# YPares/gaast

Measured on AMD Instinct MI355X. Metric: full-MV geometric products/sec (dim n); achieved HBM GB/s vs roofline, higher is better.
Workload: dtype f32; 1 GPU; R^12 full MV x MV geometric product, f32 (BASELINE configs[2]); dim=12, batch_per_gpu=65536, global_batch=65536

## Files before the change

gaast_amd/csrc/device/kernels_dense.hip.hpp:

```cpp
#pragma once
#include "kernels_common.hip.hpp"


namespace gaast {

template <typename T>
struct DenseArgs {
    const T* left;
    const T* right;
    T* out;
    int64_t left_stride, right_stride, out_stride;
    const uint32_t* left_map;
    const uint32_t* right_map;
    int left_count, right_count;
    int left_full, right_full;
    int left_contig, right_contig;
    const int32_t* out_map;
    int canon_left, canon_right;
    int n;
    uint32_t neg_hi, zero_hi;
    uint32_t neg_lo;
    int beta;
    const T* left_scale;
    const T* right_scale;
    const T* out_scale;
    const T* pre_left;
    const T* pre_right;
    int64_t pre_left_stride, pre_right_stride;
    int pre_left_len, pre_right_len, pre_canon_left, pre_canon_right;
    const uint32_t* pre_row_start;
    const uint32_t* pre_entries;
    const T* pre_coeff;
    const uint32_t* pre_row_map;
    const T* pre_row_scale;
    int pre_rows;
    int pre_width;
    int pre_scratch;
    int left_signs;
    int out_signs;
    int64_t batch;
};

__device__ __forceinline__ int dense_lds_pos(int m) {
    const int x = m >> 4, lo = m & 15;
    return (x << 4) | ((((lo >> 2) ^ (x >> 2)) & 3) << 2) | (lo & 3);
}


__device__ __forceinline__ void split_index(int e, int cnt, float inv_cnt, int nitems, int& it, int& j) {
    if (nitems == 1) {
        it = 0;
        j = e;
        return;
    }
    int q = int(float(e) * inv_cnt);
    int r = e - q * cnt;
    if (r < 0) {
        --q;
        r += cnt;
    }
    if (r >= cnt) {
        ++q;
        r -= cnt;
    }
    it = q;
    j = r;
}

template <typename T, int THREADS>
__device__ __forceinline__ void stage_operands(const T* __restrict__ src, int64_t stride, const uint32_t* __restrict__ map,
                                               int count, int contig4, int canon, T* __restrict__ images,
                                               int image_stride, int nitems, int tid, const T* __restrict__ scale = nullptr) {
    constexpr int U = 4;
    const float inv_count = 1.0f / float(count > 0 ? count : 1);
    if (contig4) {
        const int total4 = (nitems * count) >> 2;
        const int count4 = count >> 2;
        const float inv_count4 = 1.0f / float(count4 > 0 ? count4 : 1);
        for (int e0 = tid; e0 < total4; e0 += THREADS * U) {
            uint4 m[U];
            T v[U][4];
#pragma unroll
            for (int k = 0; k < U; ++k) {
                const int e = e0 + k * THREADS;
// ... 439 lines not shown
        float16v acc;
#pragma unroll
        for (int r = 0; r < 16; ++r) acc[r] = 0.f;

        const unsigned char* As_b = reinterpret_cast<const unsigned char*>(As);
        const unsigned char* Bs_b = reinterpret_cast<const unsigned char*>(Bs);
        uint32_t bq[4];
#pragma unroll
        for (int q = 0; q < 4; ++q) bq[q] = (uint32_t(c_hi) << 7) | (uint32_t((((h << 2) | q) ^ (c_hi >> 1)) & 7) << 4);
        const uint32_t c_hi_u = uint32_t(c_hi) | 0x8000u;
        auto one_step = [&](int a_hi) {
            uint32_t sp = uint32_t(a_hi) >> 1;
            sp ^= sp >> 1;
            sp ^= sp >> 2;
            sp ^= sp >> 4;
            sp ^= sp >> 8;
            const uint32_t M = sp ^ (uint32_t(a_hi) & p.neg_hi);
            const uint32_t u = (__builtin_popcount(uint32_t(a_hi) & sp) ^
                                __builtin_popcount(uint32_t(a_hi) & p.neg_hi)) & 1u;
            const uint32_t bmask = uint32_t(__builtin_popcount(c_hi_u & (M | (u << 15)))) << 31;
            float bscale = 1.f;
            if (DEGENERATE) {
                if (uint32_t(a_hi) & ~uint32_t(c_hi) & p.zero_hi) bscale = 0.f;
            }
            float bv[16];
            const uint32_t sx = (uint32_t(a_hi) << 7) | (uint32_t((a_hi >> 1) & 7) << 4);
#pragma unroll
            for (int q = 0; q < 4; ++q) {
                const float4v v = *reinterpret_cast<const float4v*>(Bs_b + (bq[q] ^ sx));
                bv[4 * q + 0] = v.x; bv[4 * q + 1] = v.y; bv[4 * q + 2] = v.z; bv[4 * q + 3] = v.w;
            }
            const uint32_t abase = uint32_t(a_hi) << 7;
#pragma unroll
            for (int s2 = 0; s2 < 16; ++s2) {
                float a = *reinterpret_cast<const float*>(As_b + abase + aoff[s2]);
                a = __uint_as_float(__float_as_uint(a) ^ amask[s2]);
                float b = __uint_as_float(__float_as_uint(bv[s2]) ^ bmask);
                if (DEGENERATE) b *= bscale;
                acc = __builtin_amdgcn_mfma_f32_32x32x2f32(a, b, acc, 0, 0, 0);
            }
        };
        const int half = H >> 1;
        for (int t2 = 0; t2 < half; ++t2) one_step((t2 << 1) | (__builtin_popcount(uint32_t(t2)) & 1));
#pragma unroll
        for (int s2 = 0; s2 < 16; ++s2)
            amask[s2] ^= uint32_t((__builtin_popcount(uint32_t(s2)) + h) & 1) << 31;
        for (int t2 = 0; t2 < half; ++t2) one_step((t2 << 1) | ((__builtin_popcount(uint32_t(t2)) & 1) ^ 1));

        float* orow = p.out + (item0 + it) * p.out_stride;
        const int32_t* om = p.out_map + (c_hi << 5);
#pragma unroll
        for (int r = 0; r < 16; ++r) {
            const int c_lo = (r & 3) + 8 * (r >> 2) + 4 * h;
            store_result<float>(orow, om[c_lo], acc[r], p.beta, out_scale, (c_hi << 5) + c_lo);
        }
    }
}

template <int THREADS>
__device__ __forceinline__ void lds_barrier() {
    if (THREADS <= 64) {
        __builtin_amdgcn_wave_barrier();
        asm volatile("" ::: "memory");
    } else {
        asm volatile("s_waitcnt lgkmcnt(0)\n\ts_barrier" ::: "memory");
    }
}

typedef __attribute__((address_space(3))) unsigned char lds_u8;
typedef uint32_t uint4v __attribute__((ext_vector_type(4)));

__device__ __forceinline__ uint32_t xor3(uint32_t a, uint32_t b, uint32_t c) {
#if __has_builtin(__builtin_amdgcn_bitop3_b32)
    return __builtin_amdgcn_bitop3_b32(a, b, c, 0x96);
#else
    return a ^ b ^ c;
#endif
}

__device__ __forceinline__ constexpr int mfma16_k(int t) {
    constexpr int order[16] = {0, 3, 5, 6, 9, 10, 12, 15, 1, 2, 4, 7, 8, 11, 13, 14};
    return order[t];
}

template <bool DEGENERATE, int NDIM, bool SCALED = false, bool CHAINED = false>
__global__ __launch_bounds__(NDIM == 13 ? 512 : 256, NDIM <= 11 ? 2 : 1) void k_gp_mfma32p(DenseArgs<float> p) {
    const float* const left_scale = SCALED ? p.left_scale : nullptr;
    const float* const right_scale = SCALED ? p.right_scale : nullptr;
    const float* const out_scale = SCALED ? p.out_scale : nullptr;
    extern __shared__ __attribute__((aligned(16))) unsigned char smem_raw[];
    float* smem = reinterpret_cast<float*>(smem_raw);
    lds_u8* lds = (lds_u8*)smem_raw;
    constexpr int n = NDIM;
    constexpr int THREADS = NDIM == 13 ? 512 : 256;
    constexpr int N = 1 << n;
    constexpr int H = 1 << (n - 5);
    constexpr int WPI = H >> 5;
    constexpr int IPB = (THREADS >> 6) / WPI;
    constexpr int item_stride = 4 * N;
    constexpr uint32_t NEG = uint32_t(N) << 2;
    constexpr int PR = N / 4;
    constexpr int MPR = PR / THREADS;
    constexpr int ROWS = 2 * IPB;
    static_assert(MPR * ROWS == 8, "eight 16-byte pieces per thread and group");
    const int tid = threadIdx.x;
    const int64_t num_groups = (p.batch + IPB - 1) / IPB;
    const bool fast = !SCALED && !CHAINED && p.left_contig && p.right_contig && p.left_full && p.right_full;

    if (tid < 16) smem[IPB * item_stride + tid] = 0.f;

    uint32_t mw[2][MPR * 4];
    float4 pf[8];
    auto fetch = [&](int64_t g) {
        const int64_t it0 = g * IPB;
        const int cnt = int(p.batch - it0 < IPB ? p.batch - it0 : IPB);
#pragma unroll
        for (int r = 0; r < ROWS; ++r) {
            const int k = r % IPB;
            if (k < cnt) {
                const float* row = r < IPB ? p.left + (it0 + k) * p.left_stride : p.right + (it0 + k) * p.right_stride;
#pragma unroll
                for (int m = 0; m < MPR; ++m) pf[r * MPR + m] = reinterpret_cast<const float4*>(row)[tid + m * THREADS];
            }
        }
    };
    if (fast) {
#pragma unroll
        for (int m = 0; m < MPR; ++m) {
            const uint4 ml = reinterpret_cast<const uint4*>(p.left_map)[tid + m * THREADS];
            const uint4 mr = reinterpret_cast<const uint4*>(p.right_map)[tid + m * THREADS];
            mw[0][4 * m + 0] = ml.x; mw[0][4 * m + 1] = ml.y; mw[0][4 * m + 2] = ml.z; mw[0][4 * m + 3] = ml.w;
            mw[1][4 * m + 0] = mr.x; mw[1][4 * m + 1] = mr.y; mw[1][4 * m + 2] = mr.z; mw[1][4 * m + 3] = mr.w;
        }
        if (int64_t(blockIdx.x) < num_groups) fetch(blockIdx.x);
    }

    const int wave = tid >> 6, lane = tid & 63;
    const int it = wave / WPI, tile = wave - it * WPI;
    const int i = lane & 31, h = lane >> 5;
    const int c_hi = (tile << 5) | i;
    const uint32_t item_base = uint32_t(it) * uint32_t(item_stride) * 4u;

    constexpr bool ABS_A = NDIM <= 11 || (NDIM == 12 && !DEGENERATE);
    const uint32_t lds0 = ABS_A ? uint32_t(size_t(lds)) : 0u;
    uint32_t ak0[16];
#pragma unroll
    for (int t = 0; t < 16; ++t) {
        const int k = 2 * mfma16_k(t) + h;
        const int a_lo = i ^ k;
        int par = __builtin_popcount(uint32_t(a_lo & k) & p.neg_lo) & 1;
        for (int pp = 1; pp < 5; ++pp)
            if ((a_lo >> pp) & 1) par ^= __builtin_popcount(k & ((1 << pp) - 1)) & 1;
        ak0[t] = lds0 + item_base + (uint32_t(a_lo) << 2) + (par ? NEG : 0u);
    }
    const uint32_t b_base = item_base + 2u * NEG;
    constexpr uint32_t zero_block = uint32_t(IPB) * uint32_t(item_stride) * 4u;
    uint32_t bq[4];
#pragma unroll
    for (int q = 0; q < 4; ++q) {
        bq[q] = (uint32_t(c_hi) << 7) | (uint32_t((((h << 2) | q) ^ (c_hi >> 1)) & 7) << 4);
        if ((__builtin_popcount(uint32_t(c_hi)) & 1) && (((q >> 1) ^ h) & 1)) bq[q] ^= NEG;
    }
    const uint32_t c_hi_u = uint32_t(c_hi) | 0x8000u;
    auto sign_terms = [&](int a_hi, uint32_t& M, uint32_t& u) {
        uint32_t sp = uint32_t(a_hi) >> 1;
        sp ^= sp >> 1;
        sp ^= sp >> 2;
        sp ^= sp >> 4;
        sp ^= sp >> 8;
        M = sp ^ (uint32_t(a_hi) & p.neg_hi);
        u = (__builtin_popcount(uint32_t(a_hi) & sp) ^ __builtin_popcount(uint32_t(a_hi) & p.neg_hi)) & 1u;
    };
    auto block_sign = [&](int a_hi) -> uint32_t {
        uint32_t M, u;
        sign_terms(a_hi, M, u);
        return uint32_t(__builtin_popcount(c_hi_u & (M | (u << 15)))) & 1u;
    };
    constexpr int SIGN_WORDS = H <= 64 ? H / 32 : 0;
    constexpr bool XOR_STEP = NDIM == 12 && !DEGENERATE;
    if (XOR_STEP && (lds0 & ((16u << n) - 1u))) __builtin_trap();
    uint32_t dlt[XOR_STEP ? 7 : 1] = {0};
    uint32_t ud[XOR_STEP ? H / 32 : 1] = {0};
    if constexpr (XOR_STEP) {
#pragma unroll
        for (int t = 0; t < 7; ++t) {
            const uint32_t P = (2u << t) - 1u;
            uint32_t M, u;
            sign_terms(int(P), M, u);
            dlt[t] = (P << 7) ^ (((P >> 1) & 7u) << 4) ^ ((uint32_t(__builtin_popcount(uint32_t(c_hi) & M)) & 1u) << (n + 2));
        }
#pragma unroll
        for (int w = 0; w < H / 32; ++w) {
            uint32_t bits = 0;
#pragma unroll 1
            for (int b = 0; b < 32; ++b) {
                uint32_t M, u0, u1;
                sign_terms(32 * w + b, M, u0);
                sign_terms(32 * w + b + 1, M, u1);
                bits |= (u0 ^ u1) << b;
            }
            ud[w] = __builtin_amdgcn_readfirstlane(bits);
        }
    }
    uint32_t sgn[SIGN_WORDS > 0 ? SIGN_WORDS : 1] = {0};
#pragma unroll
    for (int w = 0; w < SIGN_WORDS; ++w) {
        uint32_t bits = 0;
#pragma unroll 1
        for (int b = 0; b < 32; ++b) bits |= block_sign(32 * w + b) << b;
        sgn[w] = bits;
    }

    for (int64_t g = blockIdx.x; g < num_groups; g += gridDim.x) {
        const int64_t item0 = g * IPB;
        const int nitems = int(p.batch - item0 < IPB ? p.batch - item0 : IPB);
        if (fast) {
            auto stage_row = [&](int r, bool canon) {
                const int k = r % IPB, side = r / IPB;
                if (k < nitems) {
#pragma unroll
                    for (int m = 0; m < MPR; ++m) {
                        const float4 v = pf[r * MPR + m];
                        const float x[4] = {v.x, v.y, v.z, v.w};
#pragma unroll
                        for (int c = 0; c < 4; ++c) {
                            const uint32_t w = mw[side][4 * m + c];
                            float y = x[c];
                            if (canon) y = 0.f + y;
                            const uint32_t yb = __float_as_uint(y) ^ (w & 0x80000000u);
                            const uint32_t at = uint32_t(k) * uint32_t(item_stride * 4) + (side ? 2u * NEG : 0u) + (((w >> 16) & 0x7fffu) << 2);
                            *(__attribute__((address_space(3))) uint32_t*)(lds + at) = yb;
                            *(__attribute__((address_space(3))) uint32_t*)(lds + at + NEG) = yb ^ 0x80000000u;
                        }
                    }
                }
            };
#pragma unroll
            for (int r = 0; r < ROWS; ++r) {
                if constexpr (XOR_STEP) {
                    if (r / IPB ? p.canon_right : p.canon_left) stage_row(r, true);
                    else stage_row(r, false);
                } else {
                    stage_row(r, r / IPB ? p.canon_right : p.canon_left);
                }
            }
        } else {
            if (!p.left_full || !p.right_full) {
                for (int e = tid; e < nitems * item_stride; e += THREADS) smem[e] = 0.f;
                lds_barrier<THREADS>();
            }
            if constexpr (CHAINED)
                stage_from_list<float, THREADS>(p, item0, nitems, smem, item_stride, smem + p.pre_scratch, tid);
            else
                stage_operands<float, THREADS>(p.left + item0 * p.left_stride, p.left_stride, p.left_map, p.left_count, p.left_contig,
                                           p.canon_left, smem, item_stride, nitems, tid, left_scale);
            stage_operands<float, THREADS>(p.right + item0 * p.right_stride, p.right_stride, p.right_map, p.right_count,
                                           p.right_contig, p.canon_right, smem + 2 * N, item_stride, nitems, tid, right_scale);
            lds_barrier<THREADS>();
            constexpr int quads_per_item = N >> 1;
            for (int e = tid; e < nitems * quads_per_item; e += THREADS) {
                const int sit = e / quads_per_item, j = e - sit * quads_per_item;
                const int src = sit * item_stride + (j << 2) + ((j << 2) < N ? 0 : N);
                const float4v v = *reinterpret_cast<const float4v*>(smem + src);
                *reinterpret_cast<float4v*>(smem + src + N) = -v;
            }
        }
        lds_barrier<THREADS>();
        if (fast && g + gridDim.x < num_groups) fetch(g + gridDim.x);

        if (it < nitems) {
            float16v acc;
#pragma unroll
            for (int r = 0; r < 16; ++r) acc[r] = 0.f;
            uint32_t akc[XOR_STEP ? 1 : 16];
            uint32_t (&ak)[16] = *reinterpret_cast<uint32_t (*)[16]>(XOR_STEP ? ak0 : akc);
            if constexpr (!XOR_STEP) {
#pragma unroll
                for (int t = 0; t < 16; ++t) ak[t] = ak0[t];
            }

            auto step = [&](int a_hi, int j, uint32_t sxs) {
                uint32_t bw[16], aw[16];
#pragma unroll
                for (int q = 0; q < 4; ++q) {
                    uint32_t addr = b_base + (bq[q] ^ sxs);
                    if (DEGENERATE) addr = (uint32_t(a_hi) & ~uint32_t(c_hi) & p.zero_hi) ? zero_block : addr;
                    const uint4v v = *(__attribute__((address_space(3))) const uint4v*)(lds + addr);
                    bw[4 * q + 0] = v.x; bw[4 * q + 1] = v.y; bw[4 * q + 2] = v.z; bw[4 * q + 3] = v.w;
                }
#pragma unroll
                for (int t = 0; t < 16; ++t)
                    aw[t] = ABS_A ? *(__attribute__((address_space(3))) const uint32_t*)size_t(ak[t] + uint32_t(j << 7))
                                  : *(__attribute__((address_space(3))) const uint32_t*)(lds + ak[t] + uint32_t(j << 7));
#pragma unroll
                for (int t = 0; t < 16; ++t)
                    acc = __builtin_amdgcn_mfma_f32_32x32x2f32(__uint_as_float(aw[t]), __uint_as_float(bw[t]), acc, 0, 0, 0);
                asm volatile("" ::: "memory");
            };
            if constexpr (SIGN_WORDS > 0 && NDIM <= 11) {
                uint32_t awin[4];
                uint4v qb[2];
                auto b_quad = [&](int a_hi, int q, uint32_t sxs) -> uint4v {
                    uint32_t addr = b_base + (bq[q] ^ sxs);
                    if (DEGENERATE) addr = (uint32_t(a_hi) & ~uint32_t(c_hi) & p.zero_hi) ? zero_block : addr;
                    return *(__attribute__((address_space(3))) const uint4v*)(lds + addr);
                };
                auto a_word = [&](int t, int j) -> uint32_t {
                    return ABS_A ? *(__attribute__((address_space(3))) const uint32_t*)size_t(ak[t] + uint32_t(j << 7))
                                 : *(__attribute__((address_space(3))) const uint32_t*)(lds + ak[t] + uint32_t(j << 7));
                };
                auto sx_of = [&](int a_hi) -> uint32_t {
                    uint32_t sx = __builtin_amdgcn_readfirstlane((uint32_t(a_hi) << 7) | (uint32_t((a_hi >> 1) & 7) << 4));
                    asm("" : "+s"(sx));
                    return sx;
                };
                uint32_t sxs = ((sgn[0] & 1u) << (n + 2)) | sx_of(0);
                qb[0] = b_quad(0, 0, sxs);
#pragma unroll
                for (int t = 0; t < 3; ++t) awin[t] = a_word(t, 0);
#pragma unroll
                for (int w = 0; w < SIGN_WORDS; ++w) {
                    uint32_t sw = sgn[w];
                    const uint32_t next_word_bit0 = w + 1 < SIGN_WORDS ? (sgn[w + 1 < SIGN_WORDS ? w + 1 : w] & 1u) : 0u;
#pragma unroll 1
                    for (int c = 0; c < 2; ++c) {
                        const int a0 = 32 * w + 16 * c;
#pragma unroll
                        for (int j = 0; j < 16; ++j) {
                            const int a_hi = a0 + j;
                            const uint32_t nbit = j < 15 ? (sw >> (j + 1)) & 1u : (c == 0 ? (sw >> 16) & 1u : next_word_bit0);
                            const uint32_t nsxs = (nbit << (n + 2)) | sx_of(a_hi + 1);
#pragma unroll
                            for (int t = 0; t < 16; ++t) {
                                const int m = 16 * j + t;
                                const int t3 = (t + 3) & 15, j3 = j + ((t + 3) >> 4);
                                awin[(m + 3) & 3] = a_word(t3, j3);
                                if ((t & 3) == 0) {
                                    const int q = t >> 2;
                                    qb[(q + 1) & 1] = q < 3 ? b_quad(a_hi, q + 1, sxs) : b_quad(a_hi + 1, 0, nsxs);
                                }
                                __builtin_amdgcn_sched_barrier(0);
                                const uint4v bqv = qb[(t >> 2) & 1];
                                const uint32_t bwv = (t & 3) == 0 ? bqv.x : (t & 3) == 1 ? bqv.y : (t & 3) == 2 ? bqv.z : bqv.w;
                                acc = __builtin_amdgcn_mfma_f32_32x32x2f32(__uint_as_float(awin[m & 3]), __uint_as_float(bwv), acc, 0, 0, 0);
                                __builtin_amdgcn_sched_barrier(0);
                            }
                            sxs = nsxs;
                        }
                        sw >>= 16;
#pragma unroll
                        for (int t = 0; t < 16; ++t) ak[t] += 16u << 7;
                    }
                }
            } else if constexpr (XOR_STEP) {
                uint32_t xb[4];
#pragma unroll
                for (int q = 0; q < 4; ++q) xb[q] = lds0 + (b_base | bq[q]);
#pragma unroll 1
                for (int c = 0; c < H / 64; ++c) {
                    const uint32_t udw[2] = {c == 0 ? ud[0] : ud[2], c == 0 ? ud[1] : ud[3]};
#pragma unroll
                    for (int j = 0; j < 64; ++j) {
                        uint32_t bw[16], aw[16];
#pragma unroll
                        for (int q = 0; q < 4; ++q) {
                            const uint4v v = *(__attribute__((address_space(3))) const uint4v*)size_t(xb[q]);
                            bw[4 * q + 0] = v.x; bw[4 * q + 1] = v.y; bw[4 * q + 2] = v.z; bw[4 * q + 3] = v.w;
                        }
#pragma unroll
                        for (int t = 0; t < 16; ++t)
                            aw[t] = *(__attribute__((address_space(3))) const uint32_t*)size_t(ak[t] + uint32_t(j << 7));
#pragma unroll
                        for (int t = 0; t < 16; ++t)
                            acc = __builtin_amdgcn_mfma_f32_32x32x2f32(__uint_as_float(aw[t]), __uint_as_float(bw[t]), acc, 0, 0, 0);
                        asm volatile("" ::: "memory");
                        uint32_t su = __builtin_amdgcn_readfirstlane(((udw[j >> 5] >> (j & 31)) & 1u) << (n + 2));
                        asm("" : "+s"(su));
                        const uint32_t d = dlt[j < 63 ? __builtin_ctz(~uint32_t(j)) : 6];
#pragma unroll
                        for (int q = 0; q < 4; ++q) xb[q] = xor3(xb[q], d, su);
                    }
#pragma unroll
                    for (int t = 0; t < 16; ++t) ak[t] ^= 64u << 7;
                }
            } else {
                for (int a0 = 0; a0 < H; a0 += 8) {
#pragma unroll
                    for (int j = 0; j < 8; ++j) {
                        const int a_hi = a0 + j;
                        const uint32_t sx = (uint32_t(a_hi) << 7) | (uint32_t((a_hi >> 1) & 7) << 4);
                        step(a_hi, j, (block_sign(a_hi) << (n + 2)) | sx);
                    }
#pragma unroll
                    for (int t = 0; t < 16; ++t) ak[t] += 8u << 7;
                }
            }

            float* orow = p.out + (item0 + it) * p.out_stride;
            if constexpr (XOR_STEP) {
                const int32_t* om = p.out_map + (c_hi << 5);
                int32_t ow[16];
#pragma unroll
                for (int r = 0; r < 16; ++r) ow[r] = om[(r & 3) + 8 * (r >> 2) + 4 * h];
                asm volatile("" ::: "memory");
                auto put = [&](bool signs, bool beta) {
#pragma unroll
                    for (int r = 0; r < 16; ++r) {
                        const int32_t w = ow[r];
                        if (w < 0) continue;
                        float v = acc[r];
                        if (out_scale) v = v * out_scale[(c_hi << 5) + (r & 3) + 8 * (r >> 2) + 4 * h];
                        if (signs && (w & 0x40000000)) v = beta ? -v : 0.f + (-v);
                        float* dst = orow + (signs ? w & 0x3fffffff : w);
                        *dst = beta ? *dst + v : v;
                    }
                };
                if (p.out_signs) put(true, p.beta != 0);
                else put(false, p.beta != 0);
            } else {
                const int32_t* om = p.out_map + (c_hi << 5);
#pragma unroll
                for (int r = 0; r < 16; ++r) {
                    const int c_lo = (r & 3) + 8 * (r >> 2) + 4 * h;
                    store_result<float>(orow, om[c_lo], acc[r], p.beta, out_scale, (c_hi << 5) + c_lo);
                }
            }
        }
        lds_barrier<THREADS>();
    }
}

typedef double double4m __attribute__((ext_vector_type(4)));

template <typename T>
struct Mfma16x4;
template <>
struct Mfma16x4<double> {
    typedef double4m acc_t;
    static constexpr int SHIFT = 3;
    static __device__ __forceinline__ acc_t mma(double a, double b, acc_t c) { return __builtin_amdgcn_mfma_f64_16x16x4f64(a, b, c, 0, 0, 0); }
    static __device__ __forceinline__ int row(int kq, int r) { return 4 * r + kq; }
    static constexpr bool QUAD = false;
    static __device__ __forceinline__ constexpr int k_of(int kq, int s) { return 4 * s + kq; }
    static __device__ __forceinline__ double flip(double v, uint32_t bit31) { return __hiloint2double(__double2hiint(v) ^ int(bit31), __double2loint(v)); }
};
template <>
struct Mfma16x4<float> {
    typedef float4v acc_t;
    static constexpr int SHIFT = 2;
    static __device__ __forceinline__ acc_t mma(float a, float b, acc_t c) { return __builtin_amdgcn_mfma_f32_16x16x4f32(a, b, c, 0, 0, 0); }
    static __device__ __forceinline__ int row(int kq, int r) { return 4 * kq + r; }
    static constexpr bool QUAD = true;
    static __device__ __forceinline__ constexpr int k_of(int kq, int s) {
        constexpr int tab[4][4] = {{0, 3, 5, 6}, {9, 10, 12, 15}, {1, 2, 4, 7}, {8, 11, 13, 14}};
        return tab[kq][s];
    }
    static __device__ __forceinline__ float flip(float v, uint32_t bit31) { return __uint_as_float(__float_as_uint(v) ^ bit31); }
};

template <typename T, bool DEGENERATE, int NDIM, int MODE, bool SCALED = false, bool CHAINED = false>
__global__ __launch_bounds__(64 << (NDIM - 8)) __attribute__((amdgpu_waves_per_eu(2))) void k_gp_mfma16x4(DenseArgs<T> p) {
    constexpr bool FAST = MODE >= 1;
    static_assert(!(SCALED && MODE != 0), "a rescaled basis runs on the general staging and stores");
// ... 667 lines not shown
```

gaast_amd/csrc/device/plan.cpp:

```cpp
#include "plan_internal.hpp"
#include "spinor_basis.hpp"

#include <algorithm>
#include <cmath>
#include <cstdio>
#include <cstdlib>
#include <cstring>
#include <map>
#include <stdexcept>

namespace gaast {
namespace {

struct Lowering {
    const gaast_program_desc& d;
    Plan& plan;
    BladeTable bt;
    std::vector<int> cache;
    std::map<std::pair<int, int>, int> fresh;
    std::vector<char> removed;

    Lowering(const gaast_program_desc& desc, Plan& p)
        : d(desc), plan(p), bt(desc.vec_space_dim), cache(size_t(desc.n_nodes), -1) {}

    const gaast_node_desc& node(int i) const { return d.nodes[i]; }

    const Layout& layout(BufRef r) const {
        switch (r.kind) {
        case BufKind::NODE: return plan.node_buffers[size_t(r.idx)];
        case BufKind::INPUT: return plan.input_layouts[size_t(r.idx)];
        default: return plan.out_layout;
        }
    }
    static std::pair<int, int> key(BufRef r) { return {int(r.kind), r.idx}; }
    void touch(BufRef r) { fresh.erase(key(r)); }

    bool fail(int status, const std::string& msg) {
        if (plan.error == GAAST_OK) {
            plan.error = status;
            plan.error_msg = msg;
        }
        return false;
    }
    bool ok() const { return plan.error == GAAST_OK; }

    Step& emit(Step::Kind k, BufRef res, const std::string& name) {
        plan.steps.emplace_back();
        removed.push_back(0);
        Step& s = plan.steps.back();
        s.kind = k;
        s.res = res;
        s.name = name;
        return s;
    }

    void emit_zero(BufRef buf) {
        emit(Step::ZERO, buf, "zero_fill[init_null_mv]");
        fresh[key(buf)] = int(plan.steps.size()) - 1;
    }

    BufRef store_in_cache(int id) {
        if (cache[size_t(id)] >= 0) return BufRef{BufKind::NODE, cache[size_t(id)]};
        plan.node_buffers.push_back(make_layout(node(id).vec_space_dim, node(id).minimal_grade_mask));
        const int b = int(plan.node_buffers.size()) - 1;
        cache[size_t(id)] = b;
        BufRef buf{BufKind::NODE, b};
        emit_zero(buf);
        add_to_res(buf, id);
        return buf;
    }

    bool offsets_of(BufRef res, uint64_t mask, std::vector<uint32_t>& out) {
        const Layout& l = layout(res);
        for (int k = 0; k < 64; ++k) {
            if (!((mask >> k) & 1ULL)) continue;
            if (!((l.mask >> k) & 1ULL))
                return fail(GAAST_ERR_MISSING_GRADE, "grade " + std::to_string(k) + " absent from result buffer");
            for (int64_t i = 0; i < l.grade_len(k); ++i) out.push_back(uint32_t(l.offset(k) + i));
        }
        return true;
    }

// ... 632 lines not shown
                if (!adj) return S;
                if ((adj == GAAST_PROD_ADJ_LEFT) != right) return S ^ adj_z;
                const int k = __builtin_popcount(S);
                int sign = (k * (k - 1) / 2) & 1;
                sign ^= adj == GAAST_PROD_ADJ_LEFT ? reorder_parity(adj_z, S) : reorder_parity(S, adj_z);
                long double m = 1.0L;
                for (int i = 0; i < n; ++i)
                    if (((S >> i) & 1u) && d.metric_diag[i] != 0.0) m *= (long double)d.metric_diag[i];
                *f = sign ? -m : m;
                return S;
            };
            Step& s = emit(Step::PRODUCT_DENSE, res, "product_dense[gp n=" + std::to_string(n) + "]");
            s.a = ka;
            s.b = kb;
            s.canon_a = swap_ops ? canon_r : canon_l;
            s.canon_b = swap_ops ? canon_l : canon_r;
            s.beta = beta0 ? 0 : 1;
            s.n_entries = nd.n_comp_muls;
            Step::Dense& ds = s.dense;
            ds.n = n2;
            ds.family = fam;
            ds.mfma16_quads = fam == DenseFamily::MFMA16X4 && plan.dtype == GAAST_F32;
            std::vector<int> inv(size_t(n2), 0);
            bool identity = true;
            for (int j = 0; j < n2; ++j) {
                inv[size_t(perm[size_t(j)])] = j;
                identity = identity && perm[size_t(j)] == j;
            }
            std::vector<uint32_t> new_blade(size_t(1) << n2), blade_sign(size_t(1) << n2);
            for (uint32_t S = 0; S < (1u << n2); ++S) {
                uint32_t S2 = 0, par = 0;
                for (int p = 0; p < n2; ++p) {
                    if (!((S >> p) & 1u)) continue;
                    const int q = inv[size_t(p)];
                    par ^= uint32_t(__builtin_popcount(S2 >> (q + 1))) & 1u;
                    S2 |= 1u << q;
                }
                new_blade[S] = S2;
                blade_sign[S] = par;
            }
            const int pv = frame.pivot;
            const long double gp = reduced ? (long double)d.metric_diag[pv] : 1.0L;
            auto has_p = [&](uint32_t S) { return ((S >> pv) & 1u) != 0; };
            auto tau = [&](uint32_t S) -> long double { return (__builtin_popcount(S >> (pv + 1)) & 1) ? -1.0L : 1.0L; };
            auto compress = [&](uint32_t E) -> uint32_t {
                E &= ~(1u << pv);
                return (E & ((1u << pv) - 1u)) | ((E >> (pv + 1)) << pv);
            };
            auto c_of = [&](uint32_t E) -> long double {
                const int k = __builtin_popcount(E & ~(1u << pv));
                long double v = powl(-1.0L / gp, (long double)(k / 2));
                return has_p(E) ? v * tau(E) : v;
            };
            auto t_of = [&](uint32_t S) -> long double { return tau(S) * (has_p(S) ? 1.0L : 1.0L / gp); };
            auto operand_to_frame = [&](uint32_t S, bool right, long double* factor) -> uint32_t {
                if (!reduced) {
                    *factor = 1.0L;
                    return S;
                }
                const int par = right ? frame.rpar : frame.lpar;
                const uint32_t E = par ? S ^ (1u << pv) : S;
                long double f = (par ? t_of(S) : 1.0L) * c_of(E);
                if (right && frame.lpar == 1 && has_p(E)) f = -f;
                *factor = f;
                return compress(E);
            };
            auto result_from_frame = [&](uint32_t T, long double* factor) -> uint32_t {
                if (!reduced) {
                    *factor = 1.0L;
                    return T;
                }
                if ((frame.lpar ^ frame.rpar) == 0) {
                    *factor = ((frame.lpar == 1) ? gp : 1.0L) / c_of(T);
                    return compress(T);
                }
                const uint32_t E = T ^ (1u << pv);
                *factor = tau(E) * (has_p(E) ? gp : 1.0L) / c_of(E);
                return compress(E);
            };
            auto vec_pos = [](uint32_t m) {
                const uint32_t x = m >> 4, lo = m & 15;
                return (x << 4) | ((((lo >> 2) ^ (x >> 2)) & 3) << 2) | (lo & 3);
            };
            auto mfma32p_b_pos = [](uint32_t m) {
                static const int word_of_s[16] = {0, 8, 9, 1, 10, 2, 3, 11, 12, 4, 5, 13, 6, 14, 15, 7};
                const uint32_t x = m >> 5, k = m & 31, w = uint32_t(word_of_s[k >> 1]);
                const uint32_t lq = ((k & 1) << 2) | (w >> 2);
                return (x << 5) | (((lq ^ (x >> 1)) & 7) << 2) | (w & 3);
            };
            auto mfma16d_b_pos = [](uint32_t m) {
                const uint32_t x = m >> 4, k = m & 15u;
                return (x << 4) | (k ^ (((x >> 1) & 7u) << 1));
            };
            auto mfma16q_b_pos = [](uint32_t m) {
                static const int kq_of[16] = {0, 2, 2, 0, 2, 0, 0, 2, 3, 1, 1, 3, 1, 3, 3, 1};
                static const int s_of[16] = {0, 0, 1, 1, 2, 2, 3, 3, 0, 0, 1, 1, 2, 2, 3, 3};
                const uint32_t x = m >> 4, k = m & 15u;
                return (x << 4) | (uint32_t(kq_of[k] ^ int(((x >> 2) & 1u) << 1)) << 2) | uint32_t(s_of[k]);
            };
            auto mfma7_a_pos = [](uint32_t m) { return (m & 63u) + (m >> 6) * 72u; };
            auto mfma7_b_pos = [](uint32_t m) {
                static const int kq_of[8] = {0, 2, 2, 0, 3, 1, 1, 3};
                static const int s_of[8] = {0, 0, 1, 1, 0, 0, 1, 1};
                const uint32_t v = m >> 6, bh = (m >> 3) & 7u, k = m & 7u;
                return ((uint32_t(kq_of[k]) * 16u + v * 8u + bh) << 1) | uint32_t(s_of[k]);
            };
            auto mfma_b_pos = [](uint32_t m) {
                const uint32_t x = m >> 5, k = m & 31;
                const uint32_t lq = ((k & 1) << 2) | (k >> 3);
                return (x << 5) | (((lq ^ (x >> 1)) & 7) << 2) | ((k >> 1) & 3);
            };
            auto build_map = [&](const Layout& lay, uint64_t want, uint64_t flip, bool right, std::vector<uint32_t>& map,
                                 std::vector<double>& scale, int* full, int* contig) {
                bool seq = true;
                for (int k = 0; k <= n; ++k) {
                    if (!((want >> k) & 1ULL)) continue;
                    for (uint32_t i = 0; i < bt.grade_dim[size_t(k)]; ++i) {
                        long double fa;
                        const uint32_t orig = adj_operand(bt.blade_of[size_t(k)][i], right, &fa);
                        long double f1;
                        const uint32_t R = operand_to_frame(orig, right, &f1);
                        const uint32_t blade = new_blade[R];
                        const long double factor = fa * f1 * blade_scale(frame, R);
                        uint32_t neg = uint32_t((flip >> k) & 1ULL) ^ blade_sign[R] ^ (factor < 0.0L ? 1u : 0u);
                        uint32_t pos = blade;
                        switch (fam) {
                        case DenseFamily::MFMA16X4:
                            if (right) neg ^= uint32_t(__builtin_popcount(blade >> 4) & __builtin_popcount(blade & 15u) & 1);
                            if (right) pos = ds.mfma16_quads ? mfma16q_b_pos(blade) : mfma16d_b_pos(blade);
                            break;
                        case DenseFamily::MFMA32P:
                            if (right) neg ^= uint32_t(__builtin_popcount(blade >> 5) & __builtin_popcount(blade & 31u) & 1);
                            if (right) pos = mfma32p_b_pos(blade);
                            break;
                        case DenseFamily::MFMA32: if (right) pos = mfma_b_pos(blade); break;
                        case DenseFamily::MFMA7:
                            if (right) neg ^= uint32_t(__builtin_popcount((blade >> 3) & 7u) & __builtin_popcount(blade & 7u) & 1);
                            pos = right ? mfma7_b_pos(blade) : mfma7_a_pos(blade);
                            break;
                        case DenseFamily::MFMA6: break;
                        default: pos = vec_pos(blade); break;
                        }
                        const uint32_t sgn = neg ? 0x80000000u : 0u;
                        const uint32_t off = uint32_t(lay.offset(k) + i);
                        seq = seq && off == map.size();
                        map.push_back(off | (pos << 16) | sgn);
                        scale.push_back(double(fabsl(factor)));
                    }
                }
                *full = map.size() == (size_t(1) << n2);
                *contig = seq && map.size() % 4 == 0 && !map.empty();
                if (fam == DenseFamily::MFMA6 && *full) {
                    const bool f32 = plan.dtype == GAAST_F32;
                    auto lane_of = [&](uint32_t blade) -> uint32_t {
                        const uint32_t t = blade >> 4, h = (blade >> 2) & 3u, l = blade & 3u;
                        if (!right) return f32 ? ((l >> 1) << 5) | ((l & 1u) << 4) | (t << 2) | h
                                               : ((((t >> 1) << 1) | (h >> 1)) << 4) | ((t & 1u) << 3) | (l << 1) | (h & 1u);
                        return f32 ? ((h >> 1) << 5) | ((h & 1u) << 4) | (t << 2) | l
                                   : ((((h >> 1) << 1) | (l >> 1)) << 4) | (t << 2) | ((h & 1u) << 1) | (l & 1u);
                    };
                    std::vector<uint32_t> m2(map.size());
                    std::vector<double> s2(scale.size());
                    for (size_t e = 0; e < map.size(); ++e) {
                        const uint32_t q = lane_of((map[e] >> 16) & 63u);
                        m2[q] = map[e];
                        s2[q] = scale[e];
                    }
                    map.swap(m2);
                    scale.swap(s2);
                    *contig = 0;
                }
                if (fam == DenseFamily::MFMA7 && *full) {
                    const uint32_t G = plan.dtype == GAAST_F32 ? 32u : 16u;
                    std::vector<std::vector<size_t>> bucket(G);
                    for (size_t e = 0; e < map.size(); ++e) bucket[((map[e] >> 16) & 0x7fffu) % G].push_back(e);
                    bool even = true;
                    for (const auto& b : bucket) even = even && b.size() == map.size() / G;
                    if (even) {
                        std::vector<uint32_t> m2;
                        std::vector<double> s2;
                        for (size_t r = 0; r < map.size() / G; ++r)
                            for (uint32_t k = 0; k < G; ++k) {
                                m2.push_back(map[bucket[k][r]]);
                                s2.push_back(scale[bucket[k][r]]);
                            }
                        map.swap(m2);
                        scale.swap(s2);
                        *contig = 0;
                    }
                }
            };
            build_map(kla, kwa, kfa, false, ds.left_map, ds.left_scale, &ds.left_full, &ds.left_contig);
            build_map(klb, kwb, kfb, true, ds.right_map, ds.right_scale, &ds.right_full, &ds.right_contig);
            ds.out_map.assign(size_t(1) << n2, -1);
            ds.out_scale.assign(size_t(1) << n2, 1.0);
            for (uint32_t m = 0; m < (1u << n); ++m) {
                const int g = __builtin_popcount(m);
                if (!((prod_mask >> g) & 1ULL)) continue;
                long double f1;
                const uint32_t R = result_from_frame(adj ? (m ^ adj_z) : m, &f1);
                const long double factor = f1 / blade_scale(frame, R);
                const uint32_t sgn = blade_sign[R] ^ (factor < 0.0L ? 1u : 0u);
                ds.out_map[new_blade[R]] = int32_t(uint32_t(lr.offset(g) + bt.index_of[m]) | (sgn << 30));
                ds.out_scale[new_blade[R]] = double(fabsl(factor));
            }
            ds.scaled = 0;
            for (const std::vector<double>* v : {&ds.left_scale, &ds.right_scale, &ds.out_scale})
                for (double x : *v) ds.scaled |= int(x != 1.0);
            if (!ds.scaled) {
                ds.left_scale.clear();
                ds.right_scale.clear();
                ds.out_scale.clear();
            }
            ds.out_full = lr.row_len == (int64_t(1) << n2);
            for (uint32_t m = 0; m < (1u << n2); ++m) ds.out_full = ds.out_full && ds.out_map[m] >= 0;
            for (uint32_t w : ds.left_map) ds.left_signs |= int(w >> 31);
            for (int32_t w : ds.out_map) ds.out_signs |= int(w >= 0 && (uint32_t(w) & 0x40000000u));
            const bool mfma32 = fam == DenseFamily::MFMA32 || fam == DenseFamily::MFMA32P;
            const int lo_bits = mfma32 ? 5 : fam == DenseFamily::MFMA7 ? 3 : fam == DenseFamily::MFMA6 ? 0 : 4;
            for (int j = 0; j < n2; ++j) {
                const double g = frame.metric[size_t(perm[size_t(j)])];
                if (j < lo_bits) {
                    if (g < 0.0) ds.neg_lo |= 1u << j;
                } else {
                    if (g < 0.0) ds.neg_hi |= 1u << (j - lo_bits);
                    if (g == 0.0) ds.zero_hi |= 1u << (j - lo_bits);
                }
            }
            ds.neg_lo_all = fam == DenseFamily::VECTOR_FMA && ds.neg_lo == 15u;
            ds.degenerate = ds.zero_hi != 0;
            static const char* const par_name[2] = {"even", "odd"};
            s.name = std::string(fam == DenseFamily::VECTOR_FMA ? "product_dense" : "product_dense_mfma") + "[gp n=" + std::to_string(n) +
                     (reduced ? std::string(" ") + par_name[frame.lpar] + " x " + par_name[frame.rpar] + " in Cl(" + std::to_string(n2) + ")" : std::string()) +
                     (identity ? "" : " permuted basis") + (ds.scaled ? " rescaled basis" : "") +
                     (adj == GAAST_PROD_ADJ_LEFT ? " adjoint left" : adj ? " adjoint right" : "") + "]";
            touch(res);
            return;
        }

        std::vector<gaast_comp_mul> generated;
        const gaast_comp_mul* muls = nd.comp_muls;
        uint64_t n_muls = nd.n_comp_muls;
        {
            const size_t elem = plan.dtype == GAAST_F32 ? 4 : 8;
            const size_t per_item = size_t(ll.row_len + lrr.row_len) * elem;
            const bool fits_fused_slab = ll.row_len + lrr.row_len + lr.row_len < 4096;
            if (per_item > kLdsBytes && !fits_fused_slab && plan.unsupported.empty())
                plan.unsupported = "product operands of " + std::to_string(per_item) + " bytes per item exceed the " +
                                   std::to_string(kLdsBytes) + "-byte LDS the list kernels stage them in";
            if (n_muls > kMaxListEntries && plan.unsupported.empty())
                plan.unsupported = "a comp-mul list of " + std::to_string(n_muls) + " entries exceeds this back end's table budget";
            if (!plan.unsupported.empty()) return;
        }
        if (!muls && nd.product_kind >= GAAST_PROD_ADJ_LEFT) {
            const bool right = (nd.product_kind & GAAST_PROD_ADJ_RIGHT) != 0;
            const Selection sel{nd.product_kind & 7, nullptr, nullptr};
            auto contribs = right ? iter_contribs(lmin, sel, rmin, omin) : iter_contribs(lmin, sel, omin, rmin);
            const uint64_t count = comp_mul_count(d.vec_space_dim, contribs);
            if (count > kMaxAdjointListEntries && plan.unsupported.empty())
                plan.unsupported = "a compact adjoint product whose list of " + std::to_string(count) +
                                   " entries no dense kernel takes exceeds the adjoint list budget";
            if (!plan.unsupported.empty()) return;
            std::vector<gaast_comp_mul> fwd;
            fwd.reserve(size_t(count));
            for_each_comp_mul(bt, d.metric_diag, contribs, [&](const gaast_comp_mul& m) { fwd.push_back(m); });
            generated = transpose_comp_muls(fwd.data(), fwd.size(), right, true);
            muls = generated.data();
            n_muls = generated.size();
        }
        if (!muls) {
            Selection sel{nd.product_kind, nullptr, nullptr};
            auto contribs = iter_contribs(omin, sel, lmin, rmin);
            if (comp_mul_count(d.vec_space_dim, contribs) > kMaxListEntries && plan.unsupported.empty())
                plan.unsupported = "a comp-mul list of " + std::to_string(comp_mul_count(d.vec_space_dim, contribs)) +
                                   " entries exceeds this back end's table budget";
            if (!plan.unsupported.empty()) return;
            generated.reserve(size_t(comp_mul_count(d.vec_space_dim, contribs)));
            for_each_comp_mul(bt, d.metric_diag, contribs,
                              [&](const gaast_comp_mul& m) { generated.push_back(m); });
            muls = generated.data();
            n_muls = generated.size();
        }
        if (n_muls == 0) return;
        if (ll.row_len > 65536 || lrr.row_len > 65536) throw std::runtime_error("operand row too long");

        const bool beta0 = is_fresh;
        std::vector<int32_t> row_of(size_t(lr.row_len), -1);
        std::vector<uint32_t> row_out, counts;
        if (beta0)
            for (int64_t o = 0; o < lr.row_len; ++o) {
                row_of[size_t(o)] = int32_t(row_out.size());
                row_out.push_back(uint32_t(o));
                counts.push_back(0);
            }
        std::vector<uint32_t> eo(static_cast<size_t>(n_muls), 0u);
        for (uint64_t e = 0; e < n_muls; ++e) {
            const gaast_comp_mul& m = muls[e];
            auto check = [&](const Layout& lay, uint32_t g, uint32_t i, const char* what) -> int64_t {
                if (g >= 64 || !((lay.mask >> g) & 1ULL)) {
                    fail(GAAST_ERR_MISSING_GRADE, std::string("grade absent from product ") + what);
                    return -1;
                }
                if (int64_t(i) >= lay.grade_len(int(g))) throw std::runtime_error("comp-mul index out of range");
                return lay.offset(int(g)) + i;
            };
            const int64_t lo = check(ll, m.left_grade, m.left_index, "left operand");
            const int64_t ro = check(lrr, m.right_grade, m.right_index, "right operand");
            const int64_t oo = check(lr, m.result_grade, m.result_index, "result");
            if (lo < 0 || ro < 0 || oo < 0) return;
            if (row_of[size_t(oo)] < 0) {
                row_of[size_t(oo)] = int32_t(row_out.size());
                row_out.push_back(uint32_t(oo));
                counts.push_back(0);
// ... 635 lines not shown
```

Baseline: 4.326 million products/s.

## Store B operand image in quad-plane layout for dim-12 XOR-step MFMA kernel

Changes the host-side placement of right-operand blades for the n=12 non-degenerate MFMA32P path so the four B quads sit in planes at fixed strides. The kernel then tracks two LDS base pointers (even/odd) instead of four, with the per-step XOR delta recomputed for the new layout. This is meant to cut per-iteration VGPR pressure and the address XOR work in the inner loop. It adds a host/kernel layout consistency check, and it risks different LDS bank behaviour.

```diff
diff --git a/gaast_amd/csrc/device/kernels_dense.hip.hpp b/gaast_amd/csrc/device/kernels_dense.hip.hpp
--- a/gaast_amd/csrc/device/kernels_dense.hip.hpp
+++ b/gaast_amd/csrc/device/kernels_dense.hip.hpp
@@ -1,5 +1,6 @@
 #pragma once
 #include "kernels_common.hip.hpp"
+#include "mfma32p_b_planes.hip.hpp"
 
 
 namespace gaast {
@@ -605,6 +606,8 @@
     constexpr int order[16] = {0, 3, 5, 6, 9, 10, 12, 15, 1, 2, 4, 7, 8, 11, 13, 14};
     return order[t];
 }
+static_assert(mfma16_k(1) == int(b_planes::s2_of_word(1)) && mfma16_k(7) == int(b_planes::s2_of_word(7)) && mfma16_k(8) == int(b_planes::s2_of_word(8)) &&
+              mfma16_k(14) == int(b_planes::s2_of_word(14)), "the quad-plane B image stores the words in mfma16_k order");
 
 template <bool DEGENERATE, int NDIM, bool SCALED = false, bool CHAINED = false>
 __global__ __launch_bounds__(NDIM == 13 ? 512 : 256, NDIM <= 11 ? 2 : 1) void k_gp_mfma32p(DenseArgs<float> p) {
@@ -686,11 +689,7 @@
     }
     const uint32_t c_hi_u = uint32_t(c_hi) | 0x8000u;
     auto sign_terms = [&](int a_hi, uint32_t& M, uint32_t& u) {
-        uint32_t sp = uint32_t(a_hi) >> 1;
-        sp ^= sp >> 1;
-        sp ^= sp >> 2;
-        sp ^= sp >> 4;
-        sp ^= sp >> 8;
+        const uint32_t sp = b_planes::suffix_parities(uint32_t(a_hi));
         M = sp ^ (uint32_t(a_hi) & p.neg_hi);
         u = (__builtin_popcount(uint32_t(a_hi) & sp) ^ __builtin_popcount(uint32_t(a_hi) & p.neg_hi)) & 1u;
     };
@@ -706,12 +705,8 @@
     uint32_t ud[XOR_STEP ? H / 32 : 1] = {0};
     if constexpr (XOR_STEP) {
 #pragma unroll
-        for (int t = 0; t < 7; ++t) {
-            const uint32_t P = (2u << t) - 1u;
-            uint32_t M, u;
-            sign_terms(int(P), M, u);
-            dlt[t] = (P << 7) ^ (((P >> 1) & 7u) << 4) ^ ((uint32_t(__builtin_popcount(uint32_t(c_hi) & M)) & 1u) << (n + 2));
-        }
+        for (int t = 0; t < 7; ++t) dlt[t] = b_planes::delta(t, uint32_t(c_hi), p.neg_hi);
+        static_assert(!XOR_STEP || (NEG == b_planes::kNeg && IPB == 1), "one item per workgroup, the -B image 16 KiB above +B");
 #pragma unroll
         for (int w = 0; w < H / 32; ++w) {
             uint32_t bits = 0;
@@ -876,9 +871,8 @@
                     }
                 }
             } else if constexpr (XOR_STEP) {
-                uint32_t xb[4];
-#pragma unroll
-                for (int q = 0; q < 4; ++q) xb[q] = lds0 + (b_base | bq[q]);
+                uint32_t xe = lds0 + (b_base | b_planes::xe0(uint32_t(c_hi), uint32_t(h)));
+                uint32_t xo = lds0 + (b_base | b_planes::xo0(uint32_t(c_hi), uint32_t(h)));
 #pragma unroll 1
                 for (int c = 0; c < H / 64; ++c) {
                     const uint32_t udw[2] = {c == 0 ? ud[0] : ud[2], c == 0 ? ud[1] : ud[3]};
@@ -887,7 +881,7 @@
                         uint32_t bw[16], aw[16];
 #pragma unroll
                         for (int q = 0; q < 4; ++q) {
-                            const uint4v v = *(__attribute__((address_space(3))) const uint4v*)size_t(xb[q]);
+                            const uint4v v = *(__attribute__((address_space(3))) const uint4v*)size_t((q & 2 ? xo : xe) + uint32_t(q & 1) * b_planes::kQuadStride);
                             bw[4 * q + 0] = v.x; bw[4 * q + 1] = v.y; bw[4 * q + 2] = v.z; bw[4 * q + 3] = v.w;
                         }
 #pragma unroll
@@ -900,8 +894,8 @@
                         uint32_t su = __builtin_amdgcn_readfirstlane(((udw[j >> 5] >> (j & 31)) & 1u) << (n + 2));
                         asm("" : "+s"(su));
                         const uint32_t d = dlt[j < 63 ? __builtin_ctz(~uint32_t(j)) : 6];
-#pragma unroll
-                        for (int q = 0; q < 4; ++q) xb[q] = xor3(xb[q], d, su);
+                        xe = xor3(xe, d, su);
+                        xo = xor3(xo, d, su);
                     }
 #pragma unroll
                     for (int t = 0; t < 16; ++t) ak[t] ^= 64u << 7;
diff --git a/gaast_amd/csrc/device/mfma32p_b_planes.hip.hpp b/gaast_amd/csrc/device/mfma32p_b_planes.hip.hpp
--- /dev/null
+++ b/gaast_amd/csrc/device/mfma32p_b_planes.hip.hpp
@@ -0,0 +1,74 @@
+#pragma once
+
+#include <cstdint>
+
+#if defined(__HIP__) || defined(__CUDACC__)
+#define GAAST_BP_FN __host__ __device__ inline constexpr
+#else
+#define GAAST_BP_FN inline constexpr
+#endif
+
+namespace gaast {
+namespace b_planes {
+
+constexpr int kDim = 12;
+constexpr uint32_t kImageBytes = 4u << kDim;
+constexpr uint32_t kNeg = kImageBytes;
+constexpr uint32_t kQuadStride = 4096;
+constexpr uint32_t kOddQuads = 2 * kQuadStride;
+
+GAAST_BP_FN uint32_t parity(uint32_t v) {
+    v ^= v >> 16;
+    v ^= v >> 8;
+    v ^= v >> 4;
+    v ^= v >> 2;
+    v ^= v >> 1;
+    return v & 1u;
+}
+
+GAAST_BP_FN uint32_t s2_of_word(uint32_t t) {
+    constexpr uint32_t order[16] = {0, 3, 5, 6, 9, 10, 12, 15, 1, 2, 4, 7, 8, 11, 13, 14};
+    return order[t & 15u];
+}
+GAAST_BP_FN uint32_t word_of_s2(uint32_t s2) {
+    constexpr uint32_t word[16] = {0, 8, 9, 1, 10, 2, 3, 11, 12, 4, 5, 13, 6, 14, 15, 7};
+    return word[s2 & 15u];
+}
+
+GAAST_BP_FN uint32_t pos(uint32_t m) {
+    const uint32_t x = m >> 5, k = m & 31u, h = k & 1u, w = word_of_s2(k >> 1);
+    return ((w >> 2) << 10) | (h << 9) | (x << 2) | (w & 3u);
+}
+
+GAAST_BP_FN uint32_t suffix_parities(uint32_t a_hi) {
+    uint32_t sp = a_hi >> 1;
+    sp ^= sp >> 1;
+    sp ^= sp >> 2;
+    sp ^= sp >> 4;
+    sp ^= sp >> 8;
+    return sp;
+}
+GAAST_BP_FN uint32_t sign_mask(uint32_t a_hi, uint32_t neg_hi) { return suffix_parities(a_hi) ^ (a_hi & neg_hi); }
+GAAST_BP_FN uint32_t sign_uniform(uint32_t a_hi, uint32_t neg_hi) {
+    return parity(a_hi & suffix_parities(a_hi)) ^ parity(a_hi & neg_hi);
+}
+
+GAAST_BP_FN uint32_t xe0(uint32_t c_hi, uint32_t h) {
+    return (h << 11) | (c_hi << 4) | ((parity(c_hi) & h) ? kNeg : 0u);
+}
+GAAST_BP_FN uint32_t xo0(uint32_t c_hi, uint32_t h) { return xe0(c_hi, h) ^ kOddQuads ^ (parity(c_hi) ? kNeg : 0u); }
+
+GAAST_BP_FN uint32_t delta(int t, uint32_t c_hi, uint32_t neg_hi) {
+    const uint32_t P = (2u << t) - 1u;
+    return (P << 4) ^ (parity(c_hi & sign_mask(P, neg_hi)) ? kNeg : 0u);
+}
+GAAST_BP_FN uint32_t delta_uniform(uint32_t a_hi, uint32_t neg_hi) {
+    return (sign_uniform(a_hi, neg_hi) ^ sign_uniform(a_hi + 1u, neg_hi)) ? kNeg : 0u;
+}
+
+static_assert(word_of_s2(s2_of_word(0)) == 0 && word_of_s2(s2_of_word(5)) == 5 && word_of_s2(s2_of_word(9)) == 9 &&
+              word_of_s2(s2_of_word(15)) == 15, "word_of_s2 inverts s2_of_word");
+static_assert(pos(0xfffu) < 4096u && pos(0xfffu) != pos(0xffeu), "12-bit positions");
+
+}
+}
diff --git a/gaast_amd/csrc/device/plan.cpp b/gaast_amd/csrc/device/plan.cpp
--- a/gaast_amd/csrc/device/plan.cpp
+++ b/gaast_amd/csrc/device/plan.cpp
@@ -1,3 +1,4 @@
+#include "mfma32p_b_planes.hip.hpp"
 #include "plan_internal.hpp"
 #include "spinor_basis.hpp"
 
@@ -796,6 +797,8 @@
                 const uint32_t x = m >> 4, lo = m & 15;
                 return (x << 4) | ((((lo >> 2) ^ (x >> 2)) & 3) << 2) | (lo & 3);
             };
+            bool b_quad_planes = fam == DenseFamily::MFMA32P && n2 == b_planes::kDim;
+            for (int j = 5; j < n2; ++j) b_quad_planes = b_quad_planes && frame.metric[size_t(perm[size_t(j)])] != 0.0;
             auto mfma32p_b_pos = [](uint32_t m) {
                 static const int word_of_s[16] = {0, 8, 9, 1, 10, 2, 3, 11, 12, 4, 5, 13, 6, 14, 15, 7};
                 const uint32_t x = m >> 5, k = m & 31, w = uint32_t(word_of_s[k >> 1]);
@@ -845,7 +848,7 @@
                             break;
                         case DenseFamily::MFMA32P:
                             if (right) neg ^= uint32_t(__builtin_popcount(blade >> 5) & __builtin_popcount(blade & 31u) & 1);
-                            if (right) pos = mfma32p_b_pos(blade);
+                            if (right) pos = b_quad_planes ? b_planes::pos(blade) : mfma32p_b_pos(blade);
                             break;
                         case DenseFamily::MFMA32: if (right) pos = mfma_b_pos(blade); break;
                         case DenseFamily::MFMA7:
@@ -943,6 +946,10 @@
             }
             ds.neg_lo_all = fam == DenseFamily::VECTOR_FMA && ds.neg_lo == 15u;
             ds.degenerate = ds.zero_hi != 0;
+            if (b_quad_planes != (fam == DenseFamily::MFMA32P && n2 == b_planes::kDim && !ds.degenerate)) {
+                fail(GAAST_ERR_INVALID_PROGRAM, "B image layout and kernel instantiation disagree");
+                return;
+            }
             static const char* const par_name[2] = {"even", "odd"};
             s.name = std::string(fam == DenseFamily::VECTOR_FMA ? "product_dense" : "product_dense_mfma") + "[gp n=" + std::to_string(n) +
                      (reduced ? std::string(" ") + par_name[frame.lpar] + " x " + par_name[frame.rpar] + " in Cl(" + std::to_string(n2) + ")" : std::string()) +
```

Result: faster. 4.379 million products/s, median of 6 (+1.2%).
